# godk1122/IsaacLab

Measured on AMD Instinct MI355X. Metric: env-steps/sec (whole node), Anymal-C rough 4096 envs/GPU, RSL-RL PPO iteration (collect+GAE+update), higher is better.
Workload: dtype f32; 1 GPU; Isaac-Velocity-Rough-Anymal-C-v0, 4096 envs/GPU, T=24, 5 epochs x 4 minibatches, terrain 1204008 triangles, 4 state snapshots resident in HBM; parallelism=dp1, rollout=hipGraph, full_step=False, update=hipGraph (measured eager 16.93 ms, graph 16.29 ms), policy_params=571801

## Files before the change

### include/imx.h

```cpp
#ifndef IMX_H_
#define IMX_H_

#include <stddef.h>
#include <stdint.h>

#ifdef __cplusplus
extern "C" {
#endif

typedef struct imx_plan imx_plan_t;
typedef struct imx_mesh imx_mesh_t;
typedef void* imx_stream_t;

#define IMX_MAGIC 0x31584D49
#define IMX_PLAN_VERSION 3
#define IMX_HEADER_WORDS 48
#define IMX_MAX_OBS_GROUPS 4
#define IMX_REC_WORDS 20
#define IMX_FRAME_WORDS 9
#define IMX_FT_HEADER_WORDS 4

enum imx_header_word {
    IMX_H_MAGIC = 0, IMX_H_VERSION, IMX_H_J, IMX_H_B, IMX_H_H, IMX_H_A, IMX_H_D, IMX_H_R, IMX_H_NTERM, IMX_H_NREW,
    IMX_H_NOBS, IMX_H_NACT, IMX_H_MAX_EP_LEN, IMX_H_STEP_DT , IMX_H_TERM_OFF, IMX_H_REW_OFF, IMX_H_OBS_OFF,
// ... 517 lines not shown
int imx_reduce_batch_flush(imx_reduce_batch_t* batch, imx_stream_t stream);

int imx_mlp_dw_elu(int64_t M, int N, int K, const float* dH_d, int64_t ldg, const float* H_d, int64_t ldh, float elu_alpha,
                   float* dZ_out_d, int64_t ldd, const float* X_d, int64_t ldx, float* dW_d, float* db_d, void* scratch_d,
                   size_t scratch_bytes, imx_stream_t stream);

int imx_mlp_infer(int64_t M, const float* X_d, int64_t ldx, int nnets, const int* nlayers, const int* dims,
                  const float* const* weights_d, const int* weight_pitch, const float* const* biases_d, const float* elu_alpha,
                  float* const* out_d, imx_stream_t stream);

typedef struct imx_policy_act {
    const float* std_d;
    uint64_t seed;
    const int32_t* step_counter_d;
    float* actions_out_d;
    float* logp_out_d;
    float* mu_out_d;
    float* sigma_out_d;
    float* obs_out_d;
    const imx_plan_t* plan;
    const imx_state_t* state;
    const imx_buffers_t* buf;
    float pre_clip;
} imx_policy_act_t;
int imx_mlp_infer_act(int64_t M, const float* X_d, int64_t ldx, int nnets, const int* nlayers, const int* dims,
                      const float* const* weights_d, const int* weight_pitch, const float* const* packed_weights_d,
                      const float* const* biases_d, const float* elu_alpha, float* const* out_d, const imx_policy_act_t* act,
                      imx_stream_t stream);
size_t imx_mlp_packed_floats(int out_features, int in_features);
int imx_mlp_pack_weights(int out_features, int in_features, const float* W_d, int64_t ldw, float* packed_d, imx_stream_t stream);
int imx_mlp_pack_weights_batch(int nlayers, const int* out_features, const int* in_features, const float* const* W_d, const int64_t* ldw,
                               float* const* packed_d, imx_stream_t stream);

int imx_mlp_fwd_elu(int64_t M, int N, int K, const float* X_d, int64_t ldx, const float* W_d, const float* b_d, float elu_alpha,
                    int apply_elu, float* Y_d, int64_t ldy, imx_stream_t stream);

int imx_mlp_head_fwd(int64_t M, int K, int A, float* h_d, int64_t ldh, const float* W_d, const float* b_d, float* y_d,
                     int elu_in_place, float elu_alpha, imx_stream_t stream);

typedef struct imx_head_loss {
    int mode;
    int sigma_stride;
    int use_clipped_value_loss;
    float clip_param, value_loss_coef, entropy_coef, grad_scale;
    const float* sigma_d;
    const float* actions_d;
    const float* old_logp_d;
    const float* advantages_d;
    const float* returns_d;
    const float* old_values_d;
    float* dmu_d;
    float* dsigma_d;
    float* dvalue_d;
} imx_head_loss_t;
int imx_mlp_head_fwd_loss(int64_t M, int K, int A, float* h_d, int64_t ldh, const float* W_d, const float* b_d, float* y_d,
                          int elu_in_place, float elu_alpha, const imx_head_loss_t* loss, imx_stream_t stream);

int imx_mlp_head_bwd(int64_t M, int K, int A, const float* dY_d, const float* h_d, int64_t ldh, const float* W_d, float elu_alpha,
                     int has_activation, float* dprev_d, float* dW_d, float* db_d, void* scratch_d, size_t scratch_bytes,
                     imx_stream_t stream);

int imx_mlp_head_fwd_bwd(int64_t M, int K, int A, const float* z_d, int64_t ldz, const float* W_d, const float* b_d, float* y_d,
                         int elu_in, float elu_alpha, const imx_head_loss_t* loss, float* dprev_d, float* dW_d, float* db_d,
                         void* scratch_d, size_t scratch_bytes, imx_reduce_batch_t* defer_to, imx_stream_t stream);


int imx_reset_events(int64_t N, int64_t J, const uint8_t* reset_mask_d, const float* ranges28, int joint_mode,
                     const float* default_root_state_d, const float* env_origins_d, const float* default_joint_pos_d,
                     const float* default_joint_vel_d, const float* soft_joint_pos_limits_d, const float* soft_joint_vel_limits_d,
                     const float* uniforms_d, uint64_t seed, const int32_t* step_counter_d, float* root_pose_d, float* root_vel_d,
                     float* joint_pos_d, float* joint_vel_d, imx_stream_t stream);

int imx_push_velocity(int64_t N, const uint8_t* mask_d, const float* ranges12, const float* uniforms_d, uint64_t seed,
                      const int32_t* step_counter_d, float* root_vel_w_d, imx_stream_t stream);

int imx_external_force_torque(int64_t N, int64_t num_bodies, const uint8_t* mask_d, const int32_t* body_ids_d, int64_t num_ids,
                              const float* ranges4, const float* uniforms_d, uint64_t seed, const int32_t* step_counter_d,
                              float* forces_d, float* torques_d, imx_stream_t stream);

int imx_terrain_levels(int64_t N, int64_t num_levels, int64_t num_types, const uint8_t* mask_d, const float* root_pos_w_d,
                       const float* command_d, const float* terrain_origins_d, const int64_t* terrain_types_d, float terrain_size_x,
                       float max_episode_length_s, const int64_t* rand_levels_d, uint64_t seed, const int32_t* step_counter_d,
                       int64_t* terrain_levels_d, float* env_origins_d, float* mean_level_d, imx_stream_t stream);

#define IMX_IK_MAX_JOINTS 8
enum imx_ik_command { IMX_IK_POSITION = 0, IMX_IK_POSE = 1 };
enum imx_ik_method { IMX_IK_DLS = 0, IMX_IK_TRANS = 1 };
typedef struct imx_diff_ik {
    int32_t command_type;
    int32_t use_relative_mode;
    int32_t ik_method;
    int32_t has_offset;
    float lambda_val;
    float k_val;
    float offset_pos[3];
    float offset_rot[4];
    int32_t body_idx;
    int32_t jacobi_body_idx;
    int32_t num_joints;
    int32_t joint_ids[IMX_IK_MAX_JOINTS];
    int32_t jacobi_joint_ids[IMX_IK_MAX_JOINTS];
    int32_t processed_col;
} imx_diff_ik_t;

int imx_diff_ik(const imx_diff_ik_t* cfg, int64_t N, int mode, const float* processed_action_d, int64_t PA,
                const float* root_pos_w_d, const float* root_quat_w_d, const float* body_pos_w_d, const float* body_quat_w_d,
                int64_t num_bodies, const float* jacobians_d, int64_t NB, int64_t ND, const float* joint_pos_d, int64_t J,
                float* ee_pos_des_d, float* ee_quat_des_d, float* joint_pos_des_d, int64_t ld_des, imx_stream_t stream);

// ... 29 lines not shown
```

### isaaclab_amd/csrc/mlp.hip

```cpp
#include <algorithm>

#include "imx_internal.h"
#include "imx_infer_device.h"


namespace {

constexpr int DW_T = 128;
constexpr int DW_BM = 32;
constexpr int DW_LD = DW_T + 32;

struct DwArgs {
    int64_t M;
    int N, K;
    const float* dY;
    int64_t ldy;
    const float* X;
    int64_t ldx;
    float* part;
    float* part_db;
    int tn, tk, S;
    int64_t rps;
    const float* H;
    int64_t ldh;
// ... 281 lines not shown
    const int64_t i = (int64_t)(blockIdx.x - g.first_block) * 64 + tx;
    const float* src = nullptr;
    int64_t stride = 0;
    float* dst = nullptr;
    if (i < g.total) {
        src = g.part + i; stride = g.total; dst = g.out + i;
    } else if (g.db && i - g.total < g.N) {
        src = g.part_db + (i - g.total); stride = g.N; dst = g.db + (i - g.total);
    }
    float acc = 0.0f;
    if (src)
        for (int s = ty; s < g.S; s += RED_Y) acc += src[(size_t)s * stride];
    red[ty][tx] = acc;
    __syncthreads();
    if (ty == 0 && dst) {
        float sum = 0.0f;
#pragma unroll
        for (int y = 0; y < RED_Y; ++y) sum += red[y][tx];
        *dst = sum;
    }
}

struct DwPlan {
    int tn, tk, S;
    int64_t rps;
};

int g_num_cu = 0;
int g_dw_cu_budget = 0;

DwPlan dw_plan(int64_t M, int N, int K) {
    if (g_num_cu == 0) {
        int dev = 0, cu = 0;
        if (hipGetDevice(&dev) != hipSuccess || hipDeviceGetAttribute(&cu, hipDeviceAttributeMultiprocessorCount, dev) != hipSuccess || cu <= 0)
            cu = 256;
        g_num_cu = cu;
    }
    DwPlan p;
    p.tn = (N + DW_T - 1) / DW_T;
    p.tk = (K + DW_T - 1) / DW_T;
    const int T = p.tn * p.tk;
    const int cus = g_dw_cu_budget > 0 ? std::min(g_dw_cu_budget, g_num_cu) : g_num_cu;
    int64_t S = std::max<int64_t>(1, (int64_t)cus / T);
    S = std::min<int64_t>(S, std::max<int64_t>(1, M / (2 * DW_BM)));
    if (S >= 8) S &= ~(int64_t)7;
    p.rps = ((M + S - 1) / S + DW_BM - 1) / DW_BM * DW_BM;
    p.S = (int)((M + p.rps - 1) / p.rps);
    return p;
}

constexpr int HEAD_A = 64;

#define IMX_HALF_LOG_2PI_F 0.91893853320467274178f
template <bool ELU_IN, int AMAX, int LOSS>
__global__ void __launch_bounds__(256) k_head_fwd(int64_t M, int K, int A, float* __restrict__ h, int64_t ldh,
                                                  const float* __restrict__ W, const float* __restrict__ b, float* __restrict__ y,
                                                  float alpha, imx_head_loss_t L) {
    extern __shared__ float sW[];
    for (int i = threadIdx.x; i < A * K; i += blockDim.x) sW[i] = W[i];
    __syncthreads();
    const int q = threadIdx.x & 3;
    const int64_t row = (int64_t)blockIdx.x * 64 + (threadIdx.x >> 2);
    const bool live = row < M;
    float acc[AMAX];
#pragma unroll
    for (int o = 0; o < AMAX; ++o) acc[o] = 0.0f;
    float* hr = h + (live ? row : 0) * ldh;
    for (int k = 4 * q; k < K; k += 16) {
        float4 hv = *reinterpret_cast<const float4*>(hr + k);
        if (ELU_IN) {
            const float ex = (expf(fminf(hv.x, 0.0f)) - 1.0f) * alpha, ey = (expf(fminf(hv.y, 0.0f)) - 1.0f) * alpha;
            const float ez = (expf(fminf(hv.z, 0.0f)) - 1.0f) * alpha, ew = (expf(fminf(hv.w, 0.0f)) - 1.0f) * alpha;
            hv.x = hv.x > 0.0f ? hv.x : ex; hv.y = hv.y > 0.0f ? hv.y : ey; hv.z = hv.z > 0.0f ? hv.z : ez; hv.w = hv.w > 0.0f ? hv.w : ew;
            if (live) *reinterpret_cast<float4*>(hr + k) = hv;
        }
#pragma unroll
        for (int o = 0; o < AMAX; ++o)
            if (o < A) {
                const float4 wv = *reinterpret_cast<const float4*>(sW + o * K + k);
                acc[o] = fmaf(hv.w, wv.w, fmaf(hv.z, wv.z, fmaf(hv.y, wv.y, fmaf(hv.x, wv.x, acc[o]))));
            }
    }
#pragma unroll
    for (int o = 0; o < AMAX; ++o) {
        float v = acc[o];
        v += __shfl_xor(v, 1);
        v += __shfl_xor(v, 2);
        acc[o] = v + b[o < A ? o : 0];
    }
    if (q == 0 && live) {
#pragma unroll
        for (int o = 0; o < AMAX; ++o)
            if (o < A) y[row * A + o] = acc[o];
        if (LOSS == 1) {
            const float inv_m = L.grad_scale / (float)M;
            float logp = 0.0f;
#pragma unroll
            for (int o = 0; o < AMAX; ++o)
                if (o < A) {
                    const float m = acc[o], s = L.sigma_d[row * L.sigma_stride + o];
                    const float d = L.actions_d[row * A + o] - m;
                    logp += -(d * d) / (2.0f * s * s) - logf(s) - IMX_HALF_LOG_2PI_F;
                }
            const float ratio = expf(logp - L.old_logp_d[row]);
            const float ad = L.advantages_d[row], clip = L.clip_param;
            const float s1 = -ad * ratio, s2 = -ad * fminf(fmaxf(ratio, 1.0f - clip), 1.0f + clip);
            float dsur_dlogp;
            if (s1 >= s2) dsur_dlogp = -ad * ratio;
            else dsur_dlogp = (ratio > 1.0f - clip && ratio < 1.0f + clip) ? -ad * ratio : 0.0f;
            const float g = dsur_dlogp * inv_m;
#pragma unroll
            for (int o = 0; o < AMAX; ++o)
                if (o < A) {
                    const float m = acc[o], s = L.sigma_d[row * L.sigma_stride + o];
                    const float d = L.actions_d[row * A + o] - m;
                    L.dmu_d[row * A + o] = g * (d / (s * s));
                    L.dsigma_d[row * A + o] = g * ((d * d) / (s * s * s) - 1.0f / s) - L.entropy_coef * inv_m / s;
                }
        } else if (LOSS == 2) {
            const float inv_m = L.grad_scale / (float)M;
            const float v = acc[0], R = L.returns_d[row], clip = L.clip_param;
            float dv;
            if (L.use_clipped_value_loss) {
                const float vo = L.old_values_d[row];
                const float dlt = v - vo;
                const float vc = vo + fminf(fmaxf(dlt, -clip), clip);
                const float l1 = (v - R) * (v - R), l2 = (vc - R) * (vc - R);
                if (l1 >= l2) dv = 2.0f * (v - R);
                else dv = (dlt > -clip && dlt < clip) ? 2.0f * (vc - R) : 0.0f;
            } else {
                dv = -2.0f * (R - v);
            }
            L.dvalue_d[row] = L.value_loss_coef * dv * inv_m;
        }
    }
}

template <int AB>
__global__ void __launch_bounds__(512) k_head_bwd(int64_t M, int K, int A, const float* __restrict__ dY, const float* __restrict__ h,
                                                    int64_t ldh, const float* __restrict__ W, float alpha, int has_act,
                                                    float* __restrict__ dprev, float* __restrict__ part, float* __restrict__ part_db) {
    const int lane = threadIdx.x & 63, kb = threadIdx.x >> 6, r = lane & 31, half = lane >> 5;
    const int kc = kb * 32 + r;
    const int steps = (A + 1) >> 1;
    float wreg[AB * 16];
#pragma unroll
    for (int s = 0; s < AB * 16; ++s) {
        const int o = 2 * s + half;
        wreg[s] = (s < steps && o < A) ? W[o * K + kc] : 0.0f;
    }
    f32x16 wacc[AB];
    float dbacc[AB];
#pragma unroll
    for (int b = 0; b < AB; ++b) {
        dbacc[b] = 0.0f;
#pragma unroll
        for (int q = 0; q < 16; ++q) wacc[b][q] = 0.0f;
    }
    __shared__ float sdy[2][32 * (HEAD_A + 1)];
    const int P = A | 1;
    const int64_t nblk = (M + 31) / 32;
    int buf = 0;
    for (int64_t rb = blockIdx.x; rb < nblk; rb += gridDim.x, buf ^= 1) {
        const int64_t m0 = rb * 32;
        {
            const int64_t base = m0 * A, lim = M * (int64_t)A;
            for (int e = threadIdx.x; e < 32 * A; e += blockDim.x) {
                const int row = e / A, col = e - row * A;
                sdy[buf][row * P + col] = base + e < lim ? dY[base + e] : 0.0f;
            }
        }
        __syncthreads();
        const float* __restrict__ ty = sdy[buf];
        float hv[16];
#pragma unroll
        for (int q = 0; q < 16; ++q) {
            const int64_t row = m0 + acc_row(q, half);
            hv[q] = row < M ? h[row * ldh + kc] : 0.0f;
        }
        f32x16 dx;
#pragma unroll
        for (int q = 0; q < 16; ++q) dx[q] = 0.0f;
#pragma unroll
        for (int s = 0; s < AB * 16; ++s)
            if (s < steps) {
                const int o = 2 * s + half;
// ... 386 lines not shown
}

extern "C" void imx_reduce_batch_destroy(imx_reduce_batch_t* b) {
    if (t_batch == b) t_batch = nullptr;
    delete b;
}

extern "C" int imx_reduce_batch_begin(imx_reduce_batch_t* b) {
    IMX_REQUIRE(b, "imx_reduce_batch_begin: null batch");
    IMX_REQUIRE(t_batch == nullptr, "imx_reduce_batch_begin: another batch is still open on this thread (flush it first)");
    t_batch = b;
    return 0;
}

extern "C" int imx_reduce_batch_flush(imx_reduce_batch_t* b, imx_stream_t stream) {
    IMX_REQUIRE(b && t_batch == b, "imx_reduce_batch_flush: this batch is not the one open on this thread");
    t_batch = nullptr;
    if (b->args.n == 0) return 0;
    hipLaunchKernelGGL(k_mlp_reduce_batch, dim3(b->blocks), dim3(64, RED_Y), 0, (hipStream_t)stream, b->args);
    b->args.n = 0;
    b->blocks = 0;
    IMX_HIP(hipGetLastError());
    return 0;
}

extern "C" int imx_mlp_dw(int64_t M, int N, int K, const float* dY_d, int64_t ldy, const float* X_d, int64_t ldx, float* dW_d,
                          float* db_d, void* scratch_d, size_t scratch_bytes, imx_stream_t stream) {
    return mlp_dw_launch("imx_mlp_dw", M, N, K, dY_d, ldy, nullptr, 0, 0.0f, nullptr, 0, X_d, ldx, dW_d, db_d, scratch_d, scratch_bytes,
                         stream);
}

extern "C" int imx_mlp_dw_elu(int64_t M, int N, int K, const float* dH_d, int64_t ldg, const float* H_d, int64_t ldh, float elu_alpha,
                              float* dZ_out_d, int64_t ldd, const float* X_d, int64_t ldx, float* dW_d, float* db_d, void* scratch_d,
                              size_t scratch_bytes, imx_stream_t stream) {
    IMX_REQUIRE(H_d, "imx_mlp_dw_elu: the saved activation output is required");
    return mlp_dw_launch("imx_mlp_dw_elu", M, N, K, dH_d, ldg, H_d, ldh, elu_alpha, dZ_out_d, ldd, X_d, ldx, dW_d, db_d, scratch_d,
                         scratch_bytes, stream);
}

static int head_fwd_launch(int64_t M, int K, int A, float* h_d, int64_t ldh, const float* W_d, const float* b_d, float* y_d,
                           int elu_in_place, float elu_alpha, const imx_head_loss_t* loss, imx_stream_t stream) {
    IMX_REQUIRE(M > 0 && h_d && W_d && b_d && y_d, "imx_mlp_head_fwd: bad arguments");
    IMX_REQUIRE(A >= 1 && A <= HEAD_A, "imx_mlp_head_fwd: %d outputs (1..%d supported; wider layers are library GEMMs)", A, HEAD_A);
    IMX_REQUIRE(K >= 16 && K % 16 == 0 && K <= 2048 && ldh >= K && ldh % 4 == 0 && aligned16(h_d),
                "imx_mlp_head_fwd: in-features %d (pitch %lld) must be a multiple of 16, 16-byte aligned rows", K, (long long)ldh);
    IMX_REQUIRE((size_t)A * K * sizeof(float) <= 64 * 1024, "imx_mlp_head_fwd: %d x %d weights do not fit the 64 KB of LDS used", A, K);
    imx_head_loss_t L{};
    int mode = 0;
    if (loss) {
        L = *loss;
        mode = L.mode;
        IMX_REQUIRE(mode == 1 || mode == 2, "imx_mlp_head_fwd_loss: mode %d (1 policy, 2 value)", mode);
        if (mode == 1) {
            IMX_REQUIRE(L.sigma_d && L.actions_d && L.old_logp_d && L.advantages_d && L.dmu_d && L.dsigma_d, "imx_mlp_head_fwd_loss: null policy argument");
            IMX_REQUIRE(L.sigma_stride == 0 || L.sigma_stride == A, "imx_mlp_head_fwd_loss: sigma_stride must be 0 (shared std) or A");
        } else {
            IMX_REQUIRE(A == 1 && L.returns_d && L.dvalue_d && (!L.use_clipped_value_loss || L.old_values_d), "imx_mlp_head_fwd_loss: value head needs A = 1, returns, old values");
        }
    }
    const dim3 grid((unsigned)((M + 63) / 64)), block(256);
    const size_t lds = (size_t)A * K * sizeof(float);
    hipStream_t st = (hipStream_t)stream;
#define IMX_HEAD_FWD(E, AM, LS) hipLaunchKernelGGL((k_head_fwd<E, AM, LS>), grid, block, lds, st, M, K, A, h_d, ldh, W_d, b_d, y_d, elu_alpha, L)
#define IMX_HEAD_FWD_E(AM, LS) do { if (elu_in_place) IMX_HEAD_FWD(true, AM, LS); else IMX_HEAD_FWD(false, AM, LS); } while (0)
    if (A <= 16) {
        if (mode == 0) IMX_HEAD_FWD_E(16, 0); else if (mode == 1) IMX_HEAD_FWD_E(16, 1); else IMX_HEAD_FWD_E(16, 2);
    } else {
        if (mode == 0) IMX_HEAD_FWD_E(HEAD_A, 0); else if (mode == 1) IMX_HEAD_FWD_E(HEAD_A, 1); else IMX_HEAD_FWD_E(HEAD_A, 2);
    }
#undef IMX_HEAD_FWD_E
#undef IMX_HEAD_FWD
    IMX_HIP(hipGetLastError());
    return 0;
}

extern "C" int imx_mlp_head_fwd(int64_t M, int K, int A, float* h_d, int64_t ldh, const float* W_d, const float* b_d, float* y_d,
                                int elu_in_place, float elu_alpha, imx_stream_t stream) {
    return head_fwd_launch(M, K, A, h_d, ldh, W_d, b_d, y_d, elu_in_place, elu_alpha, nullptr, stream);
}

extern "C" int imx_mlp_head_fwd_loss(int64_t M, int K, int A, float* h_d, int64_t ldh, const float* W_d, const float* b_d, float* y_d,
                                     int elu_in_place, float elu_alpha, const imx_head_loss_t* loss, imx_stream_t stream) {
    IMX_REQUIRE(loss, "imx_mlp_head_fwd_loss: null loss description");
    return head_fwd_launch(M, K, A, h_d, ldh, W_d, b_d, y_d, elu_in_place, elu_alpha, loss, stream);
}

extern "C" int imx_mlp_head_bwd(int64_t M, int K, int A, const float* dY_d, const float* h_d, int64_t ldh, const float* W_d, float elu_alpha,
                                int has_activation, float* dprev_d, float* dW_d, float* db_d, void* scratch_d, size_t scratch_bytes,
                                imx_stream_t stream) {
    IMX_REQUIRE(M > 0 && dY_d && h_d && W_d && dprev_d && dW_d && db_d && scratch_d, "imx_mlp_head_bwd: bad arguments");
    IMX_REQUIRE(A >= 1 && A <= HEAD_A, "imx_mlp_head_bwd: %d outputs (1..%d supported)", A, HEAD_A);
    IMX_REQUIRE(K >= 32 && K % 32 == 0 && K <= 256 && ldh >= K, "imx_mlp_head_bwd: in-features %d must be a multiple of 32, at most 256", K);
    const int G = head_grid(M);
    const size_t need = ((size_t)G * A * K + (size_t)G * A) * sizeof(float);
    IMX_REQUIRE(scratch_bytes >= need, "imx_mlp_head_bwd: scratch too small (%zu < %zu bytes)", scratch_bytes, need);
    float* part = (float*)scratch_d;
    float* part_db = part + (size_t)G * A * K;
    hipStream_t st = (hipStream_t)stream;
    if (A <= 32)
        hipLaunchKernelGGL((k_head_bwd<1>), dim3((unsigned)G), dim3((unsigned)(K / 32 * 64)), 0, st, M, K, A, dY_d, h_d, ldh, W_d, elu_alpha,
                           has_activation, dprev_d, part, part_db);
    else
        hipLaunchKernelGGL((k_head_bwd<2>), dim3((unsigned)G), dim3((unsigned)(K / 32 * 64)), 0, st, M, K, A, dY_d, h_d, ldh, W_d, elu_alpha,
                           has_activation, dprev_d, part, part_db);
    IMX_HIP(hipGetLastError());
    return reduce_or_defer("imx_mlp_head_bwd", (int64_t)A * K, G, part, dW_d, A, part_db, db_d, st);
}

extern "C" int imx_mlp_head_fwd_bwd(int64_t M, int K, int A, const float* z_d, int64_t ldz, const float* W_d, const float* b_d, float* y_d,
                                    int elu_in, float elu_alpha, const imx_head_loss_t* loss, float* dprev_d, float* dW_d, float* db_d,
                                    void* scratch_d, size_t scratch_bytes, imx_reduce_batch_t* defer_to, imx_stream_t stream) {
    IMX_REQUIRE(M > 0 && z_d && W_d && b_d && y_d && loss && dprev_d && dW_d && db_d && scratch_d, "imx_mlp_head_fwd_bwd: bad arguments");
    IMX_REQUIRE(A >= 1 && A <= HEAD_A, "imx_mlp_head_fwd_bwd: %d outputs (1..%d supported)", A, HEAD_A);
    IMX_REQUIRE((K == 128 || K == 256) && ldz >= K && ldz % 4 == 0 && aligned16(z_d),
                "imx_mlp_head_fwd_bwd: in-features %d (pitch %lld) must be 128 or 256 with 16-byte aligned rows", K, (long long)ldz);
    IMX_REQUIRE(A <= 16, "imx_mlp_head_fwd_bwd: %d outputs (at most 16: wider heads run as imx_mlp_head_fwd_loss + imx_mlp_head_bwd)", A);
    const imx_head_loss_t L = *loss;
    IMX_REQUIRE(L.mode == 1 || L.mode == 2, "imx_mlp_head_fwd_bwd: loss mode %d (1 = policy, 2 = value)", L.mode);
    if (L.mode == 1) {
        IMX_REQUIRE(L.sigma_d && L.actions_d && L.old_logp_d && L.advantages_d && L.dmu_d && L.dsigma_d, "imx_mlp_head_fwd_bwd: null policy argument");
        IMX_REQUIRE(L.sigma_stride == 0 || L.sigma_stride == A, "imx_mlp_head_fwd_bwd: sigma_stride must be 0 (shared std) or A");
    } else {
        IMX_REQUIRE(A == 1 && L.returns_d && L.dvalue_d && (!L.use_clipped_value_loss || L.old_values_d),
                    "imx_mlp_head_fwd_bwd: value head needs A = 1, returns, old values");
    }
    const int G = head_grid(M);
    const size_t need = ((size_t)G * A * K + (size_t)G * A) * sizeof(float);
    IMX_REQUIRE(scratch_bytes >= need, "imx_mlp_head_fwd_bwd: scratch too small (%zu < %zu bytes)", scratch_bytes, need);
    float* part = (float*)scratch_d;
    float* part_db = part + (size_t)G * A * K;
    hipStream_t st = (hipStream_t)stream;
// ... 275 lines not shown
```

### isaaclab_amd/csrc/rollout.hip

```cpp
#include "imx_internal.h"

struct Mom {
    float n, mean, m2;
};
IMX_DEV Mom mom_merge(Mom a, Mom b) {
    Mom r;
    r.n = a.n + b.n;
    if (r.n == 0.0f) { r.mean = 0.0f; r.m2 = 0.0f; return r; }
    const float d = b.mean - a.mean;
    r.mean = a.mean + d * (b.n / r.n);
    r.m2 = a.m2 + b.m2 + d * d * (a.n * b.n / r.n);
    return r;
}
IMX_DEV Mom mom_wave(Mom m) {
#pragma unroll
    for (int o = 32; o > 0; o >>= 1) {
        Mom b;
        b.n = __shfl_xor(m.n, o, 64);
        b.mean = __shfl_xor(m.mean, o, 64);
        b.m2 = __shfl_xor(m.m2, o, 64);
        const bool lo = ((threadIdx.x & o) == 0);
        m = lo ? mom_merge(m, b) : mom_merge(b, m);
    }
    return m;
// ... 626 lines not shown
}

extern "C" int imx_rollout_post(int64_t N, const float* reward_d, const uint8_t* terminated_d, const uint8_t* truncated_d,
                                const float* value_t_d, float gamma, int bootstrap_time_outs, float* rewards_out_d,
                                uint8_t* dones_out_d, int64_t* dones_long_d, float* cur_reward_sum_d, float* cur_ep_len_d,
                                float* ep_stats3_d, const float* log_in_d, float* log_accum_d, int num_log, imx_stream_t stream) {
    IMX_REQUIRE(N > 0 && reward_d && terminated_d && truncated_d && value_t_d && rewards_out_d && dones_out_d,
                "imx_rollout_post: bad arguments");
    IMX_REQUIRE(!log_accum_d || (log_in_d && num_log > 0), "imx_rollout_post: log accumulation needs log_in_d and num_log > 0");
    IMX_REQUIRE((cur_reward_sum_d == nullptr) == (cur_ep_len_d == nullptr), "imx_rollout_post: episode buffers come together");
    hipLaunchKernelGGL(k_rollout_post, dim3((unsigned)((N + 255) / 256)), dim3(256), 0, (hipStream_t)stream, N, reward_d,
                       terminated_d, truncated_d, value_t_d, gamma, bootstrap_time_outs, rewards_out_d, dones_out_d,
                       dones_long_d, cur_reward_sum_d, cur_ep_len_d, ep_stats3_d, log_in_d, log_accum_d, num_log);
    IMX_HIP(hipGetLastError());
    return 0;
}

#define COLSUM_BLOCKS 256
__global__ void __launch_bounds__(256)
k_colsum_part(int64_t M, int A, const float* __restrict__ x, const float* __restrict__ y, float* __restrict__ part) {
    __shared__ float s[4][64];
    const int lane = threadIdx.x & 63, wv = threadIdx.x >> 6;
    const int64_t rows = (M + COLSUM_BLOCKS - 1) / COLSUM_BLOCKS;
    const int64_t r0 = blockIdx.x * rows, r1 = min(r0 + rows, M);
    float acc = 0.0f;
    if (lane < A)
        for (int64_t r = r0 + wv; r < r1; r += 4) acc += y ? x[r * A + lane] * y[r * A + lane] : x[r * A + lane];
    s[wv][lane] = acc;
    __syncthreads();
    if (wv == 0 && lane < A) part[(size_t)blockIdx.x * 64 + lane] = (s[0][lane] + s[1][lane]) + (s[2][lane] + s[3][lane]);
}
__global__ void __launch_bounds__(64) k_colsum_final(int A, const float* __restrict__ part, float* __restrict__ out) {
    const int c = threadIdx.x;
    if (c >= A) return;
    float a0 = 0.0f, a1 = 0.0f, a2 = 0.0f, a3 = 0.0f;
    for (int b = 0; b < COLSUM_BLOCKS; b += 4) {
        a0 += part[(size_t)b * 64 + c]; a1 += part[(size_t)(b + 1) * 64 + c];
        a2 += part[(size_t)(b + 2) * 64 + c]; a3 += part[(size_t)(b + 3) * 64 + c];
    }
    out[c] = (a0 + a1) + (a2 + a3);
}

extern "C" size_t imx_colsum_scratch_bytes(void) { return (size_t)COLSUM_BLOCKS * 64 * sizeof(float); }

extern "C" int imx_colsum(int64_t M, int64_t A, const float* x_d, const float* y_d, float* out_d, void* scratch_d,
                          imx_stream_t stream) {
    IMX_REQUIRE(M > 0 && A > 0 && A <= 64 && x_d && out_d && scratch_d, "imx_colsum: bad arguments (A <= 64)");
    float* part = reinterpret_cast<float*>(scratch_d);
    hipLaunchKernelGGL(k_colsum_part, dim3(COLSUM_BLOCKS), dim3(256), 0, (hipStream_t)stream, M, (int)A, x_d, y_d, part);
    hipLaunchKernelGGL(k_colsum_final, dim3(1), dim3(64), 0, (hipStream_t)stream, (int)A, part, out_d);
    IMX_HIP(hipGetLastError());
    return 0;
}
```

### isaaclab_amd/rsl_rl/ppo.py

```python

from __future__ import annotations

import ctypes
import os

import torch
import torch.distributed as dist
import torch.nn as nn
import torch.nn.functional as F

from .. import _lib
from .._lib import check, lib
from .storage import RolloutStorage


class _FusedPPOLoss(torch.autograd.Function):
    @staticmethod
    def forward(ctx, mu, sigma, value, actions, old_logp, old_mu, old_sigma, adv, ret, old_value, clip, clipped, vcoef, ecoef):
        L = lib()
        M, A = mu.shape
        mu_c, sg_c, v_c = mu.contiguous(), sigma.contiguous(), value.contiguous()
        args = [t.contiguous() for t in (actions, old_logp, old_mu, old_sigma, adv, ret, old_value)]
        actions, old_logp, old_mu, old_sigma, adv, ret, old_value = args
        out8 = torch.empty(8, device=mu.device)
# ... 107 lines not shown
                buf = torch.zeros(w.shape[0], kp, device=w.device, dtype=w.dtype)
                self._padded.append((buf, w))
                pitch.append(kp)
                wp.append(buf)
        L = lib()
        self._packed = [torch.zeros(int(L.imx_mlp_packed_floats(w.shape[0], w.shape[1])), device=w.device, dtype=w.dtype) for w in ws]
        self._wpk = (ctypes.c_void_p * len(ws))(*[b.data_ptr() for b in self._packed]) if os.getenv("IMX_INFER_PACKED", "1") != "0" else None
        nw = len(ws)
        self._pack_args = (nw, (ctypes.c_int * nw)(*[w.shape[0] for w in ws]), (ctypes.c_int * nw)(*[w.shape[1] for w in ws]),
                           (ctypes.c_void_p * nw)(*[w.data_ptr() for w in ws]), (ctypes.c_int64 * nw)(*[w.stride(0) for w in ws]),
                           (ctypes.c_void_p * nw)(*[b.data_ptr() for b in self._packed]))
        self._keep = (ws, bs, wp)
        self._nl = (ctypes.c_int * len(nl))(*nl)
        self._dims = (ctypes.c_int * len(dims))(*dims)
        self._w = (ctypes.c_void_p * len(wp))(*[w.data_ptr() for w in wp])
        self._pitch = (ctypes.c_int * len(pitch))(*pitch)
        self._b = (ctypes.c_void_p * len(bs))(*[b.data_ptr() for b in bs])
        self._alpha = (ctypes.c_float * len(alphas))(*alphas)
        self._n = len(nets)
        self._ctypes = ctypes
        self.refresh()

    @torch.no_grad()
    def refresh(self):
        if not self.ok:
            return
        for buf, w in self._padded:
            buf[:, :w.shape[1]].copy_(w)
        if self._wpk is not None:
            check(lib().imx_mlp_pack_weights_batch(*self._pack_args, _lib.current_stream(self._packed[0].device)))

    def __call__(self, x: torch.Tensor, *outs: torch.Tensor, act=None):
        if x.stride(1) != 1 or x.shape[1] != self.in_features or any(o is not None and not o.is_contiguous() for o in outs):
            raise _lib.ImxError("imx_mlp_infer needs a row-major input and contiguous outputs")
        out_p = (self._ctypes.c_void_p * self._n)(*[None if o is None else o.data_ptr() for o in outs])
        check(lib().imx_mlp_infer_act(x.shape[0], x.data_ptr(), x.stride(0), self._n, self._nl, self._dims, self._w, self._pitch, self._wpk,
                                      self._b, self._alpha, out_p, self._ctypes.byref(act) if act is not None else None,
                                      _lib.current_stream(x.device)))


HEAD_MAX_OUT = 64


def _is_head(lin: nn.Linear, x: torch.Tensor) -> bool:
    return (lin.out_features <= HEAD_MAX_OUT and lin.in_features % 32 == 0 and lin.in_features <= 256
            and x.stride(1) == 1 and x.stride(0) % 4 == 0)


FUSED_FIRST_LAYER_MAX_K = 256

FUSED_L0 = os.getenv("IMX_FUSED_L0", "1") != "0"
FUSED_HEAD = os.getenv("IMX_FUSED_HEAD", "0")
LOSS_ON_SIDE = os.getenv("IMX_LOSS_ON_SIDE", "1") == "1"


def fused_first_layer_ok(x: torch.Tensor, w: torch.Tensor) -> bool:
    return (x.is_cuda and x.dtype == torch.float32 and x.stride(1) == 1 and w.is_contiguous() and w.shape[1] == x.shape[1]
            and x.shape[1] <= FUSED_FIRST_LAYER_MAX_K and FUSED_L0)


def mlp_scratch(layers, M: int, device) -> torch.Tensor:
    n = max(int(lib().imx_mlp_scratch_bytes(M, lin.out_features, lin.in_features)) for lin, _ in layers)
    return torch.empty(n, dtype=torch.uint8, device=device)


class DeferredReductions:

    def __init__(self, layers, M: int, device):
        import ctypes

        L = lib()
        self.scratch = [torch.empty(int(L.imx_mlp_scratch_bytes(M, lin.out_features, lin.in_features)), dtype=torch.uint8, device=device)
                        for lin, _ in layers]
        h = ctypes.c_void_p()
        check(L.imx_reduce_batch_create(ctypes.byref(h)))
        self.handle = h

    def __del__(self):
        try:
            lib().imx_reduce_batch_destroy(self.handle)
        except Exception:
            pass


def _head_bwd_args(scratch, which="a"):
    mode = FUSED_HEAD
    if mode == "0" or (mode == "c" and which != "c") or (mode == "a" and which != "a"):
        return None
    if isinstance(scratch, DeferredReductions):
        return {"scratch": scratch.scratch[-1], "batch": scratch.handle}
    return {"scratch": scratch, "batch": None}


def mlp_forward(layers, x, out=None, head_loss=None, first=None):
    saved = [x]
    h = x
    pending_elu = None
    for li, (lin, act) in enumerate(layers):
        if li == 0 and first is not None:
            h = first
            saved.append(h)
            continue
        if act is None and _is_head(lin, h):
            if out is not None and li == len(layers) - 1:
                z = out
            else:
# ... 297 lines not shown
                self._critic_infer.refresh()
                self._critic_infer(critic_obs, self._last_values)
                return self._last_values
        return self.policy.evaluate(critic_obs).detach()

    def compute_returns(self, last_critic_obs):
        last_values = self._evaluate(last_critic_obs)
        self.storage.compute_returns(last_values, self.gamma, self.lam,
                                     normalize_advantage=not self.normalize_advantage_per_mini_batch)

    def broadcast_parameters(self):
        dist.broadcast(self.bucket.flat, src=0)

    time_allreduce = False
    _allreduce_events: list = []

    def reduce_parameters(self):
        if self.time_allreduce and self.device.type == "cuda":
            e0, e1 = torch.cuda.Event(enable_timing=True), torch.cuda.Event(enable_timing=True)
            e0.record()
            allreduce_mean_(self.bucket.grad, self.gpu_world_size)
            e1.record()
            self._allreduce_events.append((e0, e1))
            return
        allreduce_mean_(self.bucket.grad, self.gpu_world_size)

    def allreduce_us(self) -> dict | None:
        ev, self._allreduce_events = self._allreduce_events, []
        if not ev:
            return None
        ev[-1][1].synchronize()
        t = [a.elapsed_time(b) * 1e3 for a, b in ev]
        return {"mean": sum(t) / len(t), "max": max(t), "count": len(t)}

    def _side_stream(self):
        if not self.two_streams or self.device.type != "cuda":
            return None
        if self._side is None:
            self._side = torch.cuda.Stream(self.device)
        return self._side

    def _aux_stream(self):
        if getattr(self, "_aux", None) is None:
            self._aux = torch.cuda.Stream(self.device)
        return self._aux

    def _workspace(self, M: int, A: int):
        ws = self._ws.get((M, A))
        if ws is None:
            dev = self.device
            ws = dict(dmu=torch.empty(M, A, device=dev), dsigma=torch.empty(M, A, device=dev), dvalue=torch.empty(M, 1, device=dev),
                      scratch=torch.empty(int(lib().imx_ppo_scratch_bytes(M)), dtype=torch.uint8, device=dev),
                      colsum=torch.empty(int(lib().imx_colsum_scratch_bytes()), dtype=torch.uint8, device=dev),
                      mlp_a=DeferredReductions(self._actor_layers, M, dev), mlp_c=DeferredReductions(self._critic_layers, M, dev))
            self._ws[(M, A)] = ws
        return ws

    def minibatch_step(self, obs, critic_obs, actions, target_values, advantages, returns, old_logp, old_mu, old_sigma):
        L = lib()
        pol = self.policy
        stream = _lib.current_stream(self.device)
        M, A = actions.shape
        for name, t in (("actions", actions), ("target_values", target_values), ("advantages", advantages), ("returns", returns),
                        ("old_actions_log_prob", old_logp), ("old_mu", old_mu), ("old_sigma", old_sigma)):
            if not t.is_contiguous():
                raise _lib.ImxError(f"PPO.minibatch_step: {name} must be contiguous (shape {tuple(t.shape)}, strides {t.stride()})")
        ws = self._workspace(M, A)
        if pol.noise_std_type == "scalar":
            sigma, sstride = pol.std, 0
        else:
            sigma, sstride = None, A
        clipf, vclip = float(self.clip_param), int(self.use_clipped_value_loss)
        vcoef, ecoef = float(self.value_loss_coef), float(self.entropy_coef)

        heads = {"a": None, "c": None}

        def actor_pass(st):
            nonlocal sigma
            hl = None
            if sigma is not None:
                hl = {"loss": _lib.ImxHeadLoss(mode=1, sigma_stride=0, use_clipped_value_loss=vclip, clip_param=clipf, value_loss_coef=vcoef,
                                               entropy_coef=ecoef, grad_scale=1.0, sigma_d=sigma.data_ptr(), actions_d=actions.data_ptr(),
                                               old_logp_d=old_logp.data_ptr(), advantages_d=advantages.data_ptr(),
                                               dmu_d=ws["dmu"].data_ptr(), dsigma_d=ws["dsigma"].data_ptr())}
            if hl is not None:
                hl["bwd"] = _head_bwd_args(ws["mlp_a"], "a")
            mu, saved_a = mlp_forward(self._actor_layers, obs, head_loss=hl, first=first_a)
            heads["a"] = hl.get("dprev") if hl is not None else None
            if sigma is None:
                sigma = torch.exp(pol.log_std).expand_as(mu).contiguous()
            if hl is None or not hl.get("applied"):
                check(L.imx_ppo_loss_bwd(M, A, mu.data_ptr(), sigma.data_ptr(), sstride, actions.data_ptr(), old_logp.data_ptr(),
                                         advantages.data_ptr(), None, None, None, clipf, vclip, vcoef, ecoef, 1.0,
                                         ws["dmu"].data_ptr(), ws["dsigma"].data_ptr(), None, st))
            return mu, saved_a

        def critic_pass(st):
            hl = {"loss": _lib.ImxHeadLoss(mode=2, sigma_stride=0, use_clipped_value_loss=vclip, clip_param=clipf, value_loss_coef=vcoef,
                                           entropy_coef=ecoef, grad_scale=1.0, returns_d=returns.data_ptr(),
                                           old_values_d=target_values.data_ptr(), dvalue_d=ws["dvalue"].data_ptr())}
            hl["bwd"] = _head_bwd_args(ws["mlp_c"], "c")
            value, saved_c = mlp_forward(self._critic_layers, critic_obs, head_loss=hl, first=first_c)
            heads["c"] = hl.get("dprev")
            if not hl.get("applied"):
                check(L.imx_ppo_loss_bwd(M, A, None, None, sstride, None, None, None, returns.data_ptr(), value.data_ptr(),
                                         target_values.data_ptr(), clipf, vclip, vcoef, ecoef, 1.0, None, None, ws["dvalue"].data_ptr(), st))
            return value, saved_c

        def loss_values(mu, value, st):
            check(L.imx_ppo_loss_fwd(M, A, mu.data_ptr(), sigma.data_ptr(), sstride, actions.data_ptr(), old_logp.data_ptr(),
                                     old_mu.data_ptr(), old_sigma.data_ptr(), advantages.data_ptr(), returns.data_ptr(),
                                     value.data_ptr(), target_values.data_ptr(), clipf, vclip, vcoef, ecoef,
                                     self._out8.data_ptr(), self._stats.data_ptr(), ws["scratch"].data_ptr(), st))
            if pol.noise_std_type == "scalar" and A <= 64:
                check(L.imx_colsum(M, A, ws["dsigma"].data_ptr(), None, pol.std.grad.data_ptr(), ws["colsum"].data_ptr(), st))
            elif A <= 64:
                check(L.imx_colsum(M, A, ws["dsigma"].data_ptr(), sigma.data_ptr(), pol.log_std.grad.data_ptr(), ws["colsum"].data_ptr(), st))
            elif pol.noise_std_type == "scalar":
                torch.sum(ws["dsigma"], dim=0, out=pol.std.grad)
            else:
                torch.sum(ws["dsigma"] * sigma, dim=0, out=pol.log_std.grad)

        first_a = first_c = z0 = None
        joint_elu = None
        if self._joint0 is not None and critic_obs.data_ptr() == obs.data_ptr() and critic_obs.shape == obs.shape:
            w0, b0, H0, alpha0 = self._joint0
            if fused_first_layer_ok(obs, w0):
                z0 = torch.empty(obs.shape[0], 2 * H0, device=obs.device)
                check(L.imx_mlp_fwd_elu(obs.shape[0], 2 * H0, obs.shape[1], obs.data_ptr(), obs.stride(0), w0.data_ptr(), b0.data_ptr(),
                                        alpha0, 1, z0.data_ptr(), z0.stride(0), stream))
            else:
                z0 = torch.addmm(b0, obs, w0.t())
                joint_elu = alpha0
            first_a, first_c = z0[:, :H0], z0[:, H0:]
        side = self._side_stream()
        main = torch.cuda.current_stream(self.device)
        if side is not None:
            loss_on_side = LOSS_ON_SIDE
            aux = self._aux_stream()
            side.wait_stream(main)
            if joint_elu is not None:
                F.elu(first_a, alpha=joint_elu, inplace=True)
            mu, saved_a = actor_pass(stream)
            mu_ready = torch.cuda.Event()
            mu_ready.record(main)
            with torch.cuda.stream(side):
                if joint_elu is not None:
                    F.elu(first_c, alpha=joint_elu, inplace=True)
                value, saved_c = critic_pass(side.cuda_stream)
                value_ready = torch.cuda.Event()
                value_ready.record(side)
            if not loss_on_side:
                aux.wait_stream(main)
                aux.wait_event(value_ready)
            mlp_backward(self._actor_layers, saved_a, ws["dmu"], ws["mlp_a"], head_dprev=heads["a"])
            with torch.cuda.stream(side):
                mlp_backward(self._critic_layers, saved_c, ws["dvalue"], ws["mlp_c"], head_dprev=heads["c"])
                if loss_on_side:
                    side.wait_event(mu_ready)
                    loss_values(mu, value, side.cuda_stream)
            if not loss_on_side:
                with torch.cuda.stream(aux):
# ... 105 lines not shown
```

Before: 5.248 million env-steps/s.

## Fuse PPO loss statistics and std-gradient reduction into head forward kernels

The policy and value head forward+loss kernels now also write per-block double-precision partial sums of surrogate loss, entropy, KL, value loss and per-action dsigma. A single-block finish kernel reduces them into the loss outputs, stats accumulators and std gradient. This replaces the separate full-pass loss-forward kernel and the dsigma column-sum, and avoids writing dsigma to memory. It costs extra LDS and syncs in the head kernel. It assumes scalar std (writes pol.std.grad) and raises if the head path was not fused.

```diff
diff --git a/include/imx.h b/include/imx.h
--- a/include/imx.h
+++ b/include/imx.h
@@ -593,9 +593,16 @@
     float* dmu_d;
     float* dsigma_d;
     float* dvalue_d;
+    const float* old_mu_d;
+    const float* old_sigma_d;
+    void* loss_part_d;
 } imx_head_loss_t;
 int imx_mlp_head_fwd_loss(int64_t M, int K, int A, float* h_d, int64_t ldh, const float* W_d, const float* b_d, float* y_d,
                           int elu_in_place, float elu_alpha, const imx_head_loss_t* loss, imx_stream_t stream);
+
+size_t imx_head_loss_part_bytes(int64_t M, int A, int mode);
+int imx_ppo_loss_finish(int64_t M, int A, const void* policy_part_d, const void* value_part_d, float value_loss_coef,
+                        float entropy_coef, float* out8_d, float* accum5_d, float* std_grad_d, imx_stream_t stream);
 
 int imx_mlp_head_bwd(int64_t M, int K, int A, const float* dY_d, const float* h_d, int64_t ldh, const float* W_d, float elu_alpha,
                      int has_activation, float* dprev_d, float* dW_d, float* db_d, void* scratch_d, size_t scratch_bytes,
diff --git a/isaaclab_amd/csrc/mlp.hip b/isaaclab_amd/csrc/mlp.hip
--- a/isaaclab_amd/csrc/mlp.hip
+++ b/isaaclab_amd/csrc/mlp.hip
@@ -357,11 +357,13 @@
 constexpr int HEAD_A = 64;
 
 #define IMX_HALF_LOG_2PI_F 0.91893853320467274178f
-template <bool ELU_IN, int AMAX, int LOSS>
+constexpr int HEAD_PART_ROWS = 72;
+template <bool ELU_IN, int AMAX, int LOSS, bool PART = false>
 __global__ void __launch_bounds__(256) k_head_fwd(int64_t M, int K, int A, float* __restrict__ h, int64_t ldh,
                                                   const float* __restrict__ W, const float* __restrict__ b, float* __restrict__ y,
                                                   float alpha, imx_head_loss_t L) {
-    extern __shared__ float sW[];
+    extern __shared__ double sW64[];
+    float* const sW = reinterpret_cast<float*>(sW64);
     for (int i = threadIdx.x; i < A * K; i += blockDim.x) sW[i] = W[i];
     __syncthreads();
     const int q = threadIdx.x & 3;
@@ -393,19 +395,31 @@
         v += __shfl_xor(v, 2);
         acc[o] = v + b[o < A ? o : 0];
     }
+    const int nq = LOSS == 1 ? 3 + A : 1;
+    double* const sp = sW64 + (threadIdx.x >> 2) * nq;
+    if (PART) __syncthreads();
     if (q == 0 && live) {
 #pragma unroll
         for (int o = 0; o < AMAX; ++o)
             if (o < A) y[row * A + o] = acc[o];
         if (LOSS == 1) {
             const float inv_m = L.grad_scale / (float)M;
-            float logp = 0.0f;
+            float logp = 0.0f, ent = 0.0f, kl = 0.0f;
 #pragma unroll
             for (int o = 0; o < AMAX; ++o)
                 if (o < A) {
                     const float m = acc[o], s = L.sigma_d[row * L.sigma_stride + o];
                     const float d = L.actions_d[row * A + o] - m;
-                    logp += -(d * d) / (2.0f * s * s) - logf(s) - IMX_HALF_LOG_2PI_F;
+                    const float ls = logf(s);
+                    logp += -(d * d) / (2.0f * s * s) - ls - IMX_HALF_LOG_2PI_F;
+                    if (PART) {
+                        ent += 0.5f + IMX_HALF_LOG_2PI_F + ls;
+                        if (L.old_mu_d) {
+                            const float mo = L.old_mu_d[row * A + o], so = L.old_sigma_d[row * A + o];
+                            const float dm = mo - m;
+                            kl += logf(s / so + 1.0e-5f) + (so * so + dm * dm) / (2.0f * s * s) - 0.5f;
+                        }
+                    }
                 }
             const float ratio = expf(logp - L.old_logp_d[row]);
             const float ad = L.advantages_d[row], clip = L.clip_param;
@@ -414,18 +428,26 @@
             if (s1 >= s2) dsur_dlogp = -ad * ratio;
             else dsur_dlogp = (ratio > 1.0f - clip && ratio < 1.0f + clip) ? -ad * ratio : 0.0f;
             const float g = dsur_dlogp * inv_m;
+            const bool keep_dsigma = !PART || L.dsigma_d;
 #pragma unroll
             for (int o = 0; o < AMAX; ++o)
                 if (o < A) {
                     const float m = acc[o], s = L.sigma_d[row * L.sigma_stride + o];
                     const float d = L.actions_d[row * A + o] - m;
                     L.dmu_d[row * A + o] = g * (d / (s * s));
-                    L.dsigma_d[row * A + o] = g * ((d * d) / (s * s * s) - 1.0f / s) - L.entropy_coef * inv_m / s;
+                    const float ds = g * ((d * d) / (s * s * s) - 1.0f / s) - L.entropy_coef * inv_m / s;
+                    if (keep_dsigma) L.dsigma_d[row * A + o] = ds;
+                    if (PART) sp[3 + o] = ds;
                 }
+            if (PART) {
+                sp[0] = fmaxf(s1, s2);
+                sp[1] = ent;
+                sp[2] = kl;
+            }
         } else if (LOSS == 2) {
             const float inv_m = L.grad_scale / (float)M;
             const float v = acc[0], R = L.returns_d[row], clip = L.clip_param;
-            float dv;
+            float dv, vl;
             if (L.use_clipped_value_loss) {
                 const float vo = L.old_values_d[row];
                 const float dlt = v - vo;
@@ -433,10 +455,30 @@
                 const float l1 = (v - R) * (v - R), l2 = (vc - R) * (vc - R);
                 if (l1 >= l2) dv = 2.0f * (v - R);
                 else dv = (dlt > -clip && dlt < clip) ? 2.0f * (vc - R) : 0.0f;
+                vl = fmaxf(l1, l2);
             } else {
                 dv = -2.0f * (R - v);
+                vl = (R - v) * (R - v);
             }
             L.dvalue_d[row] = L.value_loss_coef * dv * inv_m;
+            if (PART) sp[0] = vl;
+        }
+    } else if (PART && q == 0) {
+        for (int c = 0; c < nq; ++c) sp[c] = 0.0;
+    }
+    if (PART) {
+        double* const sg = sW64 + 64 * nq;
+        double* const out = static_cast<double*>(L.loss_part_d) + (size_t)blockIdx.x * nq;
+        __syncthreads();
+        for (int i = threadIdx.x; i < 8 * nq; i += blockDim.x) {
+            const int grp = i / nq, c = i - grp * nq;
+            const double* p = sW64 + grp * 8 * nq + c;
+            sg[i] = ((p[0] + p[nq]) + (p[2 * nq] + p[3 * nq])) + ((p[4 * nq] + p[5 * nq]) + (p[6 * nq] + p[7 * nq]));
+        }
+        __syncthreads();
+        for (int c = threadIdx.x; c < nq; c += blockDim.x) {
+            const double* p = sg + c;
+            out[c] = ((p[0] + p[nq]) + (p[2 * nq] + p[3 * nq])) + ((p[4 * nq] + p[5 * nq]) + (p[6 * nq] + p[7 * nq]));
         }
     }
 }
@@ -929,22 +971,27 @@
         mode = L.mode;
         IMX_REQUIRE(mode == 1 || mode == 2, "imx_mlp_head_fwd_loss: mode %d (1 policy, 2 value)", mode);
         if (mode == 1) {
-            IMX_REQUIRE(L.sigma_d && L.actions_d && L.old_logp_d && L.advantages_d && L.dmu_d && L.dsigma_d, "imx_mlp_head_fwd_loss: null policy argument");
+            IMX_REQUIRE(L.sigma_d && L.actions_d && L.old_logp_d && L.advantages_d && L.dmu_d && (L.dsigma_d || L.loss_part_d),
+                        "imx_mlp_head_fwd_loss: null policy argument");
             IMX_REQUIRE(L.sigma_stride == 0 || L.sigma_stride == A, "imx_mlp_head_fwd_loss: sigma_stride must be 0 (shared std) or A");
+            IMX_REQUIRE((L.old_mu_d == nullptr) == (L.old_sigma_d == nullptr), "imx_mlp_head_fwd_loss: old_mu_d / old_sigma_d must come together");
         } else {
             IMX_REQUIRE(A == 1 && L.returns_d && L.dvalue_d && (!L.use_clipped_value_loss || L.old_values_d), "imx_mlp_head_fwd_loss: value head needs A = 1, returns, old values");
         }
     }
+    const bool part = L.loss_part_d != nullptr;
     const dim3 grid((unsigned)((M + 63) / 64)), block(256);
-    const size_t lds = (size_t)A * K * sizeof(float);
+    const size_t lds = std::max((size_t)A * K * sizeof(float), part ? (size_t)HEAD_PART_ROWS * (mode == 1 ? 3 + A : 1) * sizeof(double) : 0);
     hipStream_t st = (hipStream_t)stream;
-#define IMX_HEAD_FWD(E, AM, LS) hipLaunchKernelGGL((k_head_fwd<E, AM, LS>), grid, block, lds, st, M, K, A, h_d, ldh, W_d, b_d, y_d, elu_alpha, L)
-#define IMX_HEAD_FWD_E(AM, LS) do { if (elu_in_place) IMX_HEAD_FWD(true, AM, LS); else IMX_HEAD_FWD(false, AM, LS); } while (0)
+#define IMX_HEAD_FWD(E, AM, LS, P) hipLaunchKernelGGL((k_head_fwd<E, AM, LS, P>), grid, block, lds, st, M, K, A, h_d, ldh, W_d, b_d, y_d, elu_alpha, L)
+#define IMX_HEAD_FWD_E(AM, LS, P) do { if (elu_in_place) IMX_HEAD_FWD(true, AM, LS, P); else IMX_HEAD_FWD(false, AM, LS, P); } while (0)
+#define IMX_HEAD_FWD_P(AM, LS) do { if (part) IMX_HEAD_FWD_E(AM, LS, true); else IMX_HEAD_FWD_E(AM, LS, false); } while (0)
     if (A <= 16) {
-        if (mode == 0) IMX_HEAD_FWD_E(16, 0); else if (mode == 1) IMX_HEAD_FWD_E(16, 1); else IMX_HEAD_FWD_E(16, 2);
+        if (mode == 0) IMX_HEAD_FWD_E(16, 0, false); else if (mode == 1) IMX_HEAD_FWD_P(16, 1); else IMX_HEAD_FWD_P(16, 2);
     } else {
-        if (mode == 0) IMX_HEAD_FWD_E(HEAD_A, 0); else if (mode == 1) IMX_HEAD_FWD_E(HEAD_A, 1); else IMX_HEAD_FWD_E(HEAD_A, 2);
-    }
+        if (mode == 0) IMX_HEAD_FWD_E(HEAD_A, 0, false); else if (mode == 1) IMX_HEAD_FWD_P(HEAD_A, 1); else IMX_HEAD_FWD_P(HEAD_A, 2);
+    }
+#undef IMX_HEAD_FWD_P
 #undef IMX_HEAD_FWD_E
 #undef IMX_HEAD_FWD
     IMX_HIP(hipGetLastError());
@@ -954,6 +1001,11 @@
 extern "C" int imx_mlp_head_fwd(int64_t M, int K, int A, float* h_d, int64_t ldh, const float* W_d, const float* b_d, float* y_d,
                                 int elu_in_place, float elu_alpha, imx_stream_t stream) {
     return head_fwd_launch(M, K, A, h_d, ldh, W_d, b_d, y_d, elu_in_place, elu_alpha, nullptr, stream);
+}
+
+extern "C" size_t imx_head_loss_part_bytes(int64_t M, int A, int mode) {
+    if (M <= 0 || A < 1 || (mode != 1 && mode != 2)) return 0;
+    return (size_t)((M + 63) / 64) * (size_t)(mode == 1 ? 3 + A : 1) * sizeof(double);
 }
 
 extern "C" int imx_mlp_head_fwd_loss(int64_t M, int K, int A, float* h_d, int64_t ldh, const float* W_d, const float* b_d, float* y_d,
diff --git a/isaaclab_amd/csrc/rollout.hip b/isaaclab_amd/csrc/rollout.hip
--- a/isaaclab_amd/csrc/rollout.hip
+++ b/isaaclab_amd/csrc/rollout.hip
@@ -702,3 +702,60 @@
     IMX_HIP(hipGetLastError());
     return 0;
 }
+
+constexpr int FIN_THREADS = 256;
+__global__ void __launch_bounds__(FIN_THREADS)
+k_ppo_loss_finish(int nblk, int A, double inv_m, float vcoef, float ecoef, const double* __restrict__ ppart, const double* __restrict__ vpart,
+                  float* __restrict__ out8, float* __restrict__ accum, float* __restrict__ std_grad) {
+    __shared__ double red[FIN_THREADS];
+    __shared__ double tot[68];
+    const int nq = 3 + A, nc = nq + 1;
+    int ncp = 16;
+    while (ncp < nc) ncp <<= 1;
+    const int nch = FIN_THREADS / ncp;
+    const int c = threadIdx.x & (ncp - 1), ch = threadIdx.x / ncp;
+    if (c < nc) {
+        const double* src = c < nq ? ppart + c : vpart;
+        const int stride = c < nq ? nq : 1;
+        double acc = 0.0;
+        for (int r0 = ch * 8; r0 < nblk; r0 += nch * 8) {
+            double v[8];
+#pragma unroll
+            for (int k = 0; k < 8; ++k) v[k] = r0 + k < nblk ? src[(size_t)(r0 + k) * stride] : 0.0;
+            acc += ((v[0] + v[1]) + (v[2] + v[3])) + ((v[4] + v[5]) + (v[6] + v[7]));
+        }
+        red[ch * ncp + c] = acc;
+    }
+    __syncthreads();
+    if (threadIdx.x < nc) {
+        const int col = threadIdx.x;
+        double r[16];
+#pragma unroll
+        for (int k = 0; k < 16; ++k) r[k] = k < nch ? red[k * ncp + col] : 0.0;
+        const double lo = ((r[0] + r[1]) + (r[2] + r[3])) + ((r[4] + r[5]) + (r[6] + r[7]));
+        const double hi = ((r[8] + r[9]) + (r[10] + r[11])) + ((r[12] + r[13]) + (r[14] + r[15]));
+        tot[col] = lo + hi;
+        if (std_grad && col >= 3 && col < nq) std_grad[col - 3] = (float)(lo + hi);
+    }
+    __syncthreads();
+    if (threadIdx.x == 0) {
+        const double sur64 = tot[0] * inv_m, vl64 = tot[nq] * inv_m, ent64 = tot[1] * inv_m;
+        const float sur = (float)sur64, vl = (float)vl64, ent = (float)ent64, kl = (float)(tot[2] * inv_m);
+        out8[0] = sur; out8[1] = vl; out8[2] = ent; out8[3] = kl;
+        out8[4] = (float)(sur64 + (double)vcoef * vl64 - (double)ecoef * ent64);
+        if (accum) {
+            accum[0] += vl; accum[1] += sur; accum[2] += ent; accum[3] += kl; accum[4] += 1.0f;
+        }
+    }
+}
+
+extern "C" int imx_ppo_loss_finish(int64_t M, int A, const void* policy_part_d, const void* value_part_d, float value_loss_coef,
+                                   float entropy_coef, float* out8_d, float* accum5_d, float* std_grad_d, imx_stream_t stream) {
+    IMX_REQUIRE(M > 0 && A >= 1 && A <= 64, "imx_ppo_loss_finish: bad sizes M=%lld A=%d (A <= 64)", (long long)M, A);
+    IMX_REQUIRE((M + 63) / 64 <= INT32_MAX, "imx_ppo_loss_finish: M=%lld has too many rows of partial sums", (long long)M);
+    IMX_REQUIRE(policy_part_d && value_part_d && out8_d, "imx_ppo_loss_finish: null argument");
+    hipLaunchKernelGGL(k_ppo_loss_finish, dim3(1), dim3(FIN_THREADS), 0, (hipStream_t)stream, (int)((M + 63) / 64), A, 1.0 / (double)M,
+                       value_loss_coef, entropy_coef, (const double*)policy_part_d, (const double*)value_part_d, out8_d, accum5_d, std_grad_d);
+    IMX_HIP(hipGetLastError());
+    return 0;
+}
diff --git a/isaaclab_amd/rsl_rl/ppo.py b/isaaclab_amd/rsl_rl/ppo.py
--- a/isaaclab_amd/rsl_rl/ppo.py
+++ b/isaaclab_amd/rsl_rl/ppo.py
@@ -183,6 +183,12 @@
 FUSED_L0 = os.getenv("IMX_FUSED_L0", "1") != "0"
 FUSED_HEAD = os.getenv("IMX_FUSED_HEAD", "0")
 LOSS_ON_SIDE = os.getenv("IMX_LOSS_ON_SIDE", "1") == "1"
+
+
+def _head_loss_ok(layers) -> bool:
+    lin, act = layers[-1]
+    return (act is None and len(layers) > 1 and FUSED_HEAD == "0" and lin.out_features <= HEAD_MAX_OUT and lin.in_features % 32 == 0
+            and lin.in_features <= 256)
 
 
 def fused_first_layer_ok(x: torch.Tensor, w: torch.Tensor) -> bool:
@@ -586,6 +592,8 @@
             ws = dict(dmu=torch.empty(M, A, device=dev), dsigma=torch.empty(M, A, device=dev), dvalue=torch.empty(M, 1, device=dev),
                       scratch=torch.empty(int(lib().imx_ppo_scratch_bytes(M)), dtype=torch.uint8, device=dev),
                       colsum=torch.empty(int(lib().imx_colsum_scratch_bytes()), dtype=torch.uint8, device=dev),
+                      part_a=torch.empty(int(lib().imx_head_loss_part_bytes(M, A, 1)), dtype=torch.uint8, device=dev),
+                      part_c=torch.empty(int(lib().imx_head_loss_part_bytes(M, 1, 2)), dtype=torch.uint8, device=dev),
                       mlp_a=DeferredReductions(self._actor_layers, M, dev), mlp_c=DeferredReductions(self._critic_layers, M, dev))
             self._ws[(M, A)] = ws
         return ws
@@ -607,6 +615,9 @@
         clipf, vclip = float(self.clip_param), int(self.use_clipped_value_loss)
         vcoef, ecoef = float(self.value_loss_coef), float(self.entropy_coef)
 
+        partials = (sigma is not None and A <= HEAD_MAX_OUT and _head_loss_ok(self._actor_layers) and _head_loss_ok(self._critic_layers)
+                    and self._critic_layers[-1][0].out_features == 1)
+
         heads = {"a": None, "c": None}
 
         def actor_pass(st):
@@ -616,11 +627,16 @@
                 hl = {"loss": _lib.ImxHeadLoss(mode=1, sigma_stride=0, use_clipped_value_loss=vclip, clip_param=clipf, value_loss_coef=vcoef,
                                                entropy_coef=ecoef, grad_scale=1.0, sigma_d=sigma.data_ptr(), actions_d=actions.data_ptr(),
                                                old_logp_d=old_logp.data_ptr(), advantages_d=advantages.data_ptr(),
-                                               dmu_d=ws["dmu"].data_ptr(), dsigma_d=ws["dsigma"].data_ptr())}
+                                               dmu_d=ws["dmu"].data_ptr(), dsigma_d=None if partials else ws["dsigma"].data_ptr())}
+                if partials:
+                    hl["loss"].old_mu_d, hl["loss"].old_sigma_d = old_mu.data_ptr(), old_sigma.data_ptr()
+                    hl["loss"].loss_part_d = ws["part_a"].data_ptr()
             if hl is not None:
                 hl["bwd"] = _head_bwd_args(ws["mlp_a"], "a")
             mu, saved_a = mlp_forward(self._actor_layers, obs, head_loss=hl, first=first_a)
             heads["a"] = hl.get("dprev") if hl is not None else None
+            if partials and not hl.get("applied"):
+                raise _lib.ImxError("PPO.minibatch_step: the policy head did not run as imx_mlp_head_fwd_loss (no loss sums were written)")
             if sigma is None:
                 sigma = torch.exp(pol.log_std).expand_as(mu).contiguous()
             if hl is None or not hl.get("applied"):
@@ -633,15 +649,23 @@
             hl = {"loss": _lib.ImxHeadLoss(mode=2, sigma_stride=0, use_clipped_value_loss=vclip, clip_param=clipf, value_loss_coef=vcoef,
                                            entropy_coef=ecoef, grad_scale=1.0, returns_d=returns.data_ptr(),
                                            old_values_d=target_values.data_ptr(), dvalue_d=ws["dvalue"].data_ptr())}
+            if partials:
+                hl["loss"].loss_part_d = ws["part_c"].data_ptr()
             hl["bwd"] = _head_bwd_args(ws["mlp_c"], "c")
             value, saved_c = mlp_forward(self._critic_layers, critic_obs, head_loss=hl, first=first_c)
             heads["c"] = hl.get("dprev")
+            if partials and not hl.get("applied"):
+                raise _lib.ImxError("PPO.minibatch_step: the value head did not run as imx_mlp_head_fwd_loss (no loss sums were written)")
             if not hl.get("applied"):
                 check(L.imx_ppo_loss_bwd(M, A, None, None, sstride, None, None, None, returns.data_ptr(), value.data_ptr(),
                                          target_values.data_ptr(), clipf, vclip, vcoef, ecoef, 1.0, None, None, ws["dvalue"].data_ptr(), st))
             return value, saved_c
 
         def loss_values(mu, value, st):
+            if partials:
+                check(L.imx_ppo_loss_finish(M, A, ws["part_a"].data_ptr(), ws["part_c"].data_ptr(), vcoef, ecoef, self._out8.data_ptr(),
+                                            self._stats.data_ptr(), pol.std.grad.data_ptr(), st))
+                return
             check(L.imx_ppo_loss_fwd(M, A, mu.data_ptr(), sigma.data_ptr(), sstride, actions.data_ptr(), old_logp.data_ptr(),
                                      old_mu.data_ptr(), old_sigma.data_ptr(), advantages.data_ptr(), returns.data_ptr(),
                                      value.data_ptr(), target_values.data_ptr(), clipf, vclip, vcoef, ecoef,
```

Result: no change. 5.267 million env-steps/s, median of 6 (+0.4%).
